# facebookresearch/brainmagick

Measured on AMD Instinct MI355X. Metric: segments/s, 208-ch x 360-sample SimpleConv + ClipLoss training step, higher is better.
Workload: dtype f32 (fp32-accurate: operands split into 2 scaled f16 planes, 3 MFMA products, fp32 accumulate; same parity tolerances as exact fp32, see DESIGN.md §2); 1 GPU; cfg2: gwilliams2022-shaped MEG C=208 T=360, F=120 features, 27 subjects, clip_conv SimpleConv (8985590 params) + ClipLoss + Adam; batch_per_gpu=256, global_batch=256, negatives=local, parallelism=dp1, comm=none, rccl_world=1, candidate_gather=none, distinct_batches=8

## Files before the change

### brainmagick_amd/csrc/core.hip

```cpp
#include "bm_common.h"
#include <stdarg.h>
#include <stdlib.h>

thread_local char bm_err_buf[512] = {0};

int bm_set_error(int code, const char* fmt, ...) {
    va_list ap;
    va_start(ap, fmt);
    vsnprintf(bm_err_buf, sizeof(bm_err_buf), fmt, ap);
    va_end(ap);
    return code;
}

int bm_check_launch(const char* what) {
    hipError_t e = hipGetLastError();
    if (e != hipSuccess) return bm_set_error((int)e, "%s: launch failed: %s", what, hipGetErrorString(e));
    return BM_OK;
}

extern "C" const char* bm_last_error(void) { return bm_err_buf; }
extern "C" int bm_version(void) { return 110; }

extern "C" int bm_device_count(void) {
    int n = 0;
    hipError_t e = hipGetDeviceCount(&n);
    if (e != hipSuccess) { bm_set_error((int)e, "hipGetDeviceCount: %s", hipGetErrorString(e)); return -1; }
    return n;
}

__global__ __launch_bounds__(1024) void amax_finalize_kernel(const float* __restrict__ ws, int n, float* __restrict__ out) {
    __shared__ float sh[16];
    float m = 0.f;
    for (int i = threadIdx.x; i < n; i += 1024) m = fmaxf(m, ws[i]);
    m = bm_wave_max(m);
    if ((threadIdx.x & 63) == 0) sh[threadIdx.x >> 6] = m;
    __syncthreads();
    if (threadIdx.x < BM_AMAX_SHARDS) {
        float v = 0.f;
        if (threadIdx.x == 0)
            for (int w = 0; w < 16; ++w) v = fmaxf(v, sh[w]);
        out[threadIdx.x] = v;
    }
}

// ... 50 lines not shown
```

### brainmagick_amd/csrc/gemm_nt_h2w.hip

```cpp
#include <cstdlib>
#include "gemm_nt_common.h"

typedef _Float16 f16x8 __attribute__((ext_vector_type(8)));
typedef _Float16 f16x4 __attribute__((ext_vector_type(4)));
typedef unsigned int u32x2 __attribute__((ext_vector_type(2)));

#define HG_K 32
#define HG_XQ (64 + 2)

struct GemmNTArgsH {
    const float* a; long a_sstride; long a_rstride;
    const float* x; long x_sstride; long x_rstride;
    const float* a_amax; const float* x_amax;
    const float* a_row_amax;
    float* part;
    int S, M, Cn, T, dil, nsplit;
    int tiles_m, tiles_c;
    const int* order; const int* seg;
};

__device__ __forceinline__ u32x4 hg_ld128(__amdgpu_buffer_rsrc_t rs, int voff, int soff) {
    return __builtin_amdgcn_raw_buffer_load_b128(rs, voff, soff, 0);
}
__device__ __forceinline__ unsigned hg_ld32(__amdgpu_buffer_rsrc_t rs, int voff) {
    return __builtin_amdgcn_raw_buffer_load_b32(rs, voff, 0, 0);
}

__device__ __forceinline__ void hg_split_store4(const float (&f)[4], float s, char* dst, int plane_bytes) {
    f16x4 h, l;
#pragma unroll
    for (int i = 0; i < 4; ++i) {
        const float xs = f[i] * s;
        const _Float16 a = (_Float16)xs;
        h[i] = a;
        l[i] = (_Float16)(xs - (float)a);
    }
    *reinterpret_cast<u32x2*>(dst) = __builtin_bit_cast(u32x2, h);
    *reinterpret_cast<u32x2*>(dst + plane_bytes) = __builtin_bit_cast(u32x2, l);
}

__device__ __forceinline__ void hg_split_hi(float x0, float x1, float s0, float s1, unsigned& hi) {
    asm("v_fma_mixlo_f16 %0, %1, %3, 0\n\t"
// ... 21 lines not shown
                     :: "memory");
}

template <int NP>
__device__ __forceinline__ void hg_touch(u32x4 (&r)[NP]) {
    if constexpr (NP == 16)
        asm volatile("" :: "v"(r[0]), "v"(r[1]), "v"(r[2]), "v"(r[3]), "v"(r[4]), "v"(r[5]), "v"(r[6]), "v"(r[7]),
                     "v"(r[8]), "v"(r[9]), "v"(r[10]), "v"(r[11]), "v"(r[12]), "v"(r[13]), "v"(r[14]), "v"(r[15]));
    else
        asm volatile("" :: "v"(r[0]), "v"(r[1]), "v"(r[2]), "v"(r[3]), "v"(r[4]), "v"(r[5]), "v"(r[6]), "v"(r[7]),
                     "v"(r[8]), "v"(r[9]), "v"(r[10]), "v"(r[11]));
}

#ifdef HG_TRACE
__device__ long long hg_trace_buf[64 * 4 * 8];
#define HG_T(I_) { __builtin_amdgcn_sched_barrier(0); tr[I_] = __builtin_readcyclecounter(); __builtin_amdgcn_sched_barrier(0); }
extern "C" int bm_debug_trace_read(long long* out) {
    return (int)hipMemcpyFromSymbol(out, HIP_SYMBOL(hg_trace_buf), sizeof(long long) * 64 * 4 * 8);
}
#else
#define HG_T(I_)
#endif

template <int KS, int MW, int NS, bool RS = false, bool TS = false, bool FL = false>
__global__ __launch_bounds__(256, 1) void gemm_nt_h2w_kernel(GemmNTArgsH a) {
    static_assert(!FL || RS, "the flat walk relies on the row-scaled A path (pieces inside or outside a row)");
    static_assert((MW == 5 && NS == 3) || (MW == 4 && NS == 2) || (MW == 4 && NS == 4),
                  "tile variants: 320 x 192, 256 x 128, 256 x 256");
    static_assert(!TS || (KS == 1 && !RS), "the transposed partial tile is the score contraction's");
    static_assert(KS == 1 || NS == 3, "3 taps use the 3 slots");
    constexpr int NA = 2 * MW;
    constexpr int NX = 2 * NS;
    constexpr int NP = NA + NX;
    constexpr int BM = 64 * MW;
    constexpr int BC = KS == 3 ? 64 : 64 * NS;
    constexpr int AQ = BM + 2;
    constexpr int ASLOTS = 4 * AQ;
    constexpr int PLANE = ASLOTS + NS * 4 * HG_XQ;
    constexpr int BUF = 2 * PLANE;
    constexpr int TN = MW * NS;
    constexpr int NXS = KS == 3 ? 3 : 1;
#ifdef HG_TRACE
    const long long t_kernel0 = __builtin_readcyclecounter();
    long long t_loop0 = t_kernel0, t_loop1 = t_kernel0;
#endif
    extern __shared__ __attribute__((aligned(16))) float smem[];
    u32x4* lds = reinterpret_cast<u32x4*>(smem);
    const int tid = threadIdx.x;
    const int lane = tid & 63;
    const int wave = __builtin_amdgcn_readfirstlane(tid >> 6);
    const int wm = wave >> 1, wc = wave & 1;
    const int nl = lane & 31, h = lane >> 5;

    int id = bm_xcd_remap(blockIdx.x, gridDim.x);
    const int tm = id % a.tiles_m; id /= a.tiles_m;
    const int tc = id % a.tiles_c; id /= a.tiles_c;
    const int split = id % a.nsplit;
    const int grp = id / a.nsplit;
    const int m0 = tm * BM, c0 = tc * BC;
    const int s_first = a.seg ? a.seg[grp] : 0;
    const int s_count = a.seg ? a.seg[grp + 1] - s_first : a.S;
#define HG_SEG(K_) (a.order ? a.order[s_first + (K_)] : s_first + (K_))

    const int cps = (a.T + HG_K - 1) / HG_K;
    const long nchunks = FL ? ((long)a.S * a.T + HG_K - 1) / HG_K : (long)s_count * cps;
    const long q_begin = nchunks * split / a.nsplit;
    const long q_end = nchunks * (split + 1) / a.nsplit;
    const int nst = (int)(q_end - q_begin);
    const int halo = KS == 3 ? a.dil : 0;
    const int a_bytes = (int)(((FL ? (long)(a.S - 1) * a.a_sstride : 0) + (long)(a.M - 1) * a.a_rstride + a.T) * 4);
    const int x_bytes = (int)(((FL ? (long)(a.S - 1) * a.x_sstride : 0) + (long)(a.Cn - 1) * a.x_rstride + a.T) * 4);
    float sa, sa_inv, sx, sx_inv;
    bm_scale_from_amax(bm_amax_load(a.a_amax), sa, sa_inv);
    bm_scale_from_amax(bm_amax_load(a.x_amax), sx, sx_inv);

    const int row32 = tid >> 3, pl = tid & 7;
    int offa[NA], offx[NX];
#pragma unroll
    for (int i = 0; i < NA; ++i) {
        const int m = m0 + 32 * i + row32;
        offa[i] = m < a.M ? (m * (int)a.a_rstride + 4 * pl) * 4 : 0x7f000000;
    }
#pragma unroll
    for (int q = 0; q < NX; ++q) {
        const int c = c0 + (KS == 3 ? 0 : 64 * (q >> 1)) + 32 * (q & 1) + row32;
        offx[q] = c < a.Cn ? (c * (int)a.x_rstride + 4 * pl) * 4 : 0x7f000000;
    }
    const int ldsa = ((pl >> 1) * AQ + row32) * 16 + (pl & 1) * 8;
    const int ldsx = (ASLOTS + (pl >> 1) * HG_XQ + row32) * 16 + (pl & 1) * 8;

// ... 232 lines not shown
#undef HG_SV
#undef HG_S
#undef HG_SPLIT0
#undef HG_SPLIT_SUB
#undef HG_BOOKKEEPING
#undef HG_SPLIT1
#undef HG_WRITE
#undef HG_READ_A1
#undef HG_READ_B1
#undef HG_READ_A
#undef HG_READ_B

    const long N = (long)a.Cn * KS;
    float* dst = a.part + ((long)grp * a.nsplit + split) * a.M * N;
    if constexpr (RS) {
        __syncthreads();
        for (int i = tid; i < BM; i += 256) {
            float s_unused, inv_m = 0.f;
            if (m0 + i < a.M) bm_scale_from_amax(a.a_row_amax[m0 + i], s_unused, inv_m);
            smem[i] = inv_m;
        }
        __syncthreads();
    }
    if constexpr (TS) {
        const float f = sa_inv * sx_inv;
        float* dstT = a.part + ((long)grp * a.nsplit + split) * a.Cn * a.M;
#pragma unroll
        for (int j = 0; j < NS; ++j) {
            const int c = c0 + 64 * j + wc * 32 + nl;
            if (c < a.Cn) {
#pragma unroll
                for (int mt = 0; mt < MW; ++mt)
#pragma unroll
                    for (int q = 0; q < 4; ++q) {
                        const int m = m0 + wm * (MW * 32) + mt * 32 + 8 * q + 4 * h;
                        if (m < a.M)
                            *reinterpret_cast<float4*>(dstT + (long)c * a.M + m) =
                                float4{acc[mt][j][4 * q] * f, acc[mt][j][4 * q + 1] * f, acc[mt][j][4 * q + 2] * f,
                                       acc[mt][j][4 * q + 3] * f};
                    }
            }
        }
        return;
    }
#pragma unroll
    for (int mt = 0; mt < MW; ++mt) {
// ... 10 lines not shown
                        p[0] = acc[mt][0][r] * f;
                        p[1] = acc[mt][1][r] * f;
                        p[2] = acc[mt][2][r] * f;
                    }
                } else {
#pragma unroll
                    for (int j = 0; j < NS; ++j) {
                        const int c = c0 + 64 * j + wc * 32 + nl;
                        if (c < a.Cn) dst[(long)m * N + c] = acc[mt][j][r] * f;
                    }
                }
            }
        }
    }
#ifdef HG_TRACE
    asm volatile("s_waitcnt vmcnt(0)" ::: "memory");
    if (blockIdx.x < 64 && lane == 0) {
        long long* o = hg_trace_buf + (blockIdx.x * 4 + wave) * 8;
        o[2] = t_loop0 - t_kernel0;
        o[3] = t_loop1 - t_loop0;
        o[6] = (long long)__builtin_readcyclecounter() - t_loop1;
    }
#endif
}

static int hg_family(int S, int G, int M, int Cn, int T, int KS, int dil, bool ordered) {
    if (KS != 3 && KS != 1) return 0;
    if ((G != 1 || ordered) && KS != 1) return 0;
    if (dil < 1 || dil > 32 || T < 2 * HG_K) return 0;
    if ((long)S * ((T + HG_K - 1) / HG_K) < 32L * G) return 0;
    const long work = (long)M * Cn;
    const long pad53 = (long)cdiv(M, 320) * 320 * cdiv(Cn, KS == 3 ? 64 : 192) * (KS == 3 ? 64 : 192);
    if (KS == 3) return pad53 * 4 <= work * 5 ? 1 : 0;
    const long pad42 = (long)cdiv(M, 256) * 256 * cdiv(Cn, 128) * 128;
    if (pad42 < pad53 && pad42 <= work * 2) return 2;
    return pad53 <= work * 2 ? 1 : 0;
}

extern "C" int bm_gemm_nt_h2_covers(int M, int Cn, int KS, int S, int T, int G, int dil, int ordered) {
    return hg_family(S, G, M, Cn, T, KS, dil, ordered != 0) ? 1 : 0;
}

extern "C" int bm_gemm_nt_h2_suggest_splits(int M, int Cn, int KS, int S, int T) {
    return bm_gemm_nt_h2_suggest_splits_grouped(M, Cn, KS, S, T, 1);
}
extern "C" int bm_gemm_nt_h2_suggest_splits_grouped(int M, int Cn, int KS, int S, int T, int G) {
// ... 3 lines not shown
    const long chunks = (long)(S / G > 0 ? S / G : 1) * ((T + HG_K - 1) / HG_K);
    long want = 256 / tiles;
    if (want > chunks / 8) want = chunks / 8;
    if (want < 1) want = 1;
    return (int)want;
}

template <int KS, int MW, int NS, bool RS = false, bool TS = false, bool FL = false>
static int launch_gemm_nt_h2w(GemmNTArgsH g, hipStream_t stream, int ngroups = 1) {
    constexpr int PLANE = 4 * (64 * MW + 2) + NS * 4 * HG_XQ;
    const size_t lds = (size_t)2 * 2 * PLANE * 16;
    static bool attr_set = false;
    if (!attr_set) {
        hipError_t e = hipFuncSetAttribute(reinterpret_cast<const void*>(gemm_nt_h2w_kernel<KS, MW, NS, RS, TS, FL>),
                                           hipFuncAttributeMaxDynamicSharedMemorySize, (int)lds);
        if (e != hipSuccess) return bm_set_error((int)e, "gemm_nt_h2w: hipFuncSetAttribute: %s", hipGetErrorString(e));
        attr_set = true;
    }
    g.tiles_m = cdiv(g.M, 64 * MW);
    g.tiles_c = cdiv(g.Cn, KS == 3 ? 64 : 64 * NS);
    const long nblocks = (long)g.tiles_m * g.tiles_c * g.nsplit * ngroups;
    hipLaunchKernelGGL((gemm_nt_h2w_kernel<KS, MW, NS, RS, TS, FL>), dim3((unsigned)nblocks), dim3(256), lds, stream, g);
    return bm_check_launch("gemm_nt_h2w");
}

static int gemm_nt_h2_impl(const float* a, long a_sstride, long a_rstride, const float* a_amax, const float* a_row_amax,
                           const float* x, long x_sstride, long x_rstride, const float* x_amax, float* part, int S,
                           int M, int Cn, int T, int KS, int dil, int nsplit, void* stream,
                           const int* order = nullptr, const int* seg = nullptr, int G = 1) {
    BM_REQUIRE(a && x && part && a_amax && x_amax, "gemm_nt_h2: null pointer");
    BM_REQUIRE(M > 0 && Cn > 0 && T > 0 && nsplit > 0 && S >= 0, "gemm_nt_h2: bad dims");
    BM_REQUIRE(G >= 1 && (G == 1 || seg), "gemm_nt_h2: a grouped call needs seg[]");
    const bool grouped = seg != nullptr || order != nullptr;
    const int fam = hg_family(S, G, M, Cn, T, KS, dil, grouped);
    BM_REQUIRE(fam != 0, "gemm_nt_h2: shape not covered (M=%d Cn=%d T=%d KS=%d dil=%d)", M, Cn, T, KS, dil);
    if (((long)(M - 1) * a_rstride + T) * 4 >= 0x7f000000L || ((long)(Cn - 1) * x_rstride + T) * 4 >= 0x7f000000L)
        return bm_gemm_nt_x3(a, a_sstride, a_rstride, x, x_sstride, x_rstride, order, seg, part, S, G, M, Cn, T,
                             KS, dil, nsplit, stream);
    GemmNTArgsH g;
    g.a = a; g.a_sstride = a_sstride; g.a_rstride = a_rstride; g.a_amax = a_amax;
    g.x = x; g.x_sstride = x_sstride; g.x_rstride = x_rstride; g.x_amax = x_amax;
    g.a_row_amax = a_row_amax;
    g.part = part; g.S = S; g.M = M; g.Cn = Cn; g.T = T; g.dil = dil; g.nsplit = nsplit;
    g.order = order; g.seg = seg;
    hipStream_t s = (hipStream_t)stream;
    if (grouped) {
        if (fam == 2) return launch_gemm_nt_h2w<1, 4, 2>(g, s, G);
        return launch_gemm_nt_h2w<1, 5, 3>(g, s, G);
    }
    const bool rs = a_row_amax && fam == 1 && T % 4 == 0 && a_rstride % 4 == 0 && a_sstride % 4 == 0;
    const bool flat = rs && KS == 3 && T % HG_K != 0 && T >= 2 * HG_K && S > 1 &&
                      ((long)(S - 1) * a_sstride + (long)(M - 1) * a_rstride + T) * 4 < 0x7f000000L &&
                      ((long)(S - 1) * x_sstride + (long)(Cn - 1) * x_rstride + T) * 4 < 0x7f000000L &&
                      a_sstride >= T && x_sstride >= T && x_sstride % 4 == 0;
    if (flat) return launch_gemm_nt_h2w<3, 5, 3, true, false, true>(g, s);
    if (KS == 3) return rs ? launch_gemm_nt_h2w<3, 5, 3, true>(g, s) : launch_gemm_nt_h2w<3, 5, 3>(g, s);
    if (fam == 2) return launch_gemm_nt_h2w<1, 4, 2>(g, s);
    return rs ? launch_gemm_nt_h2w<1, 5, 3, true>(g, s) : launch_gemm_nt_h2w<1, 5, 3>(g, s);
}

extern "C" int bm_gemm_nt_h2(const float* a, long a_sstride, long a_rstride, const float* a_amax, const float* x,
                             long x_sstride, long x_rstride, const float* x_amax, float* part, int S, int M, int Cn,
                             int T, int KS, int dil, int nsplit, void* stream) {
    return gemm_nt_h2_impl(a, a_sstride, a_rstride, a_amax, nullptr, x, x_sstride, x_rstride, x_amax, part, S, M, Cn, T,
                           KS, dil, nsplit, stream);
}

extern "C" int bm_gemm_nt_h2_rows(const float* a, long a_sstride, long a_rstride, const float* a_amax,
                                  const float* a_row_amax, const float* x, long x_sstride, long x_rstride,
                                  const float* x_amax, float* part, int S, int M, int Cn, int T, int KS, int dil,
                                  int nsplit, void* stream) {
    return gemm_nt_h2_impl(a, a_sstride, a_rstride, a_amax, a_row_amax, x, x_sstride, x_rstride, x_amax, part, S, M, Cn,
                           T, KS, dil, nsplit, stream);
}

extern "C" int bm_gemm_nt_h2_grouped(const float* a, long a_sstride, long a_rstride, const float* a_amax, const float* x,
                                     long x_sstride, long x_rstride, const float* x_amax, const int* order,
                                     const int* seg, float* part, int S, int G, int M, int Cn, int T, int nsplit,
                                     void* stream) {
    return gemm_nt_h2_impl(a, a_sstride, a_rstride, a_amax, nullptr, x, x_sstride, x_rstride, x_amax, part, S, M, Cn, T,
                           1, 1, nsplit, stream, order, seg, G);
}

static int clip_scores_wide(int B, int Bc, long K) {
    const long tiles = (long)cdiv(Bc, 256) * cdiv(B, 256);
    const long chunks = (K + HG_K - 1) / HG_K;
    long splits = 256 / tiles;
    if (splits < 1) splits = 1;
    return chunks / splits >= 16;
}

extern "C" int bm_clip_scores_h2_covers(int B, int Bc, long K) {
    if (B <= 0 || Bc <= 0 || Bc % 4 != 0 || K < 16 * HG_K || K >= 0x7fffffffL) return 0;
    if (((long)(Bc - 1) * K + K) * 4 >= 0x7f000000L || ((long)(B - 1) * K + K) * 4 >= 0x7f000000L) return 0;
    const int bc = clip_scores_wide(B, Bc, K) ? 256 : 128;
    return (long)cdiv(Bc, 256) * 256 * cdiv(B, bc) * bc * 2 <= (long)B * Bc * 3;
}

extern "C" int bm_clip_scores_h2_suggest_splits(int B, int Bc, long K) {
    const int bc = clip_scores_wide(B, Bc, K) ? 256 : 128;
    const int tiles = cdiv(Bc, 256) * cdiv(B, bc);
    const long chunks = (K + HG_K - 1) / HG_K;
    long want = 256 / tiles;
    if (want > chunks / 4) want = chunks / 4;
// ... 17 lines not shown
```

### brainmagick_amd/functional.py

```python

import torch

from . import hip_ops as H



ACT_CODES = {"none": H.ACT_NONE, "gelu": H.ACT_GELU, "relu": H.ACT_RELU, "leaky": H.ACT_LEAKY}


def _c(t: torch.Tensor) -> torch.Tensor:
    return t if t.is_contiguous() else t.contiguous()


_arange_cache = {}


def _arange_i32(n: int, device, repeat: int = 1) -> torch.Tensor:
    key = (n, repeat, device.type, device.index)
    t = _arange_cache.get(key)
    if t is None:
        if len(_arange_cache) > 64:
            _arange_cache.clear()
        t = torch.arange(n, dtype=torch.int32, device=device)
        if repeat != 1:
            t = t.repeat(repeat)
        if device.type == "cuda":
            torch.cuda.current_stream(device).synchronize()
        _arange_cache[key] = t
    return t


def _conv_weight_grads(dy, x, weight, KS, dil, transposed_weight):
    dst = H.grad_destination(weight)
    B, M, T = dy.shape
    Cin = x.shape[1]
    if transposed_weight:
        out = dst if dst is not None else torch.empty(weight.shape, device=dy.device, dtype=torch.float32)
        H.gemm_nt(x, dy, B, Cin, M, T, 1, 1, out=out.view(1, Cin, M, 1))
        return out.view(weight.shape) if dst is not None else out
    if dst is not None:
        H.gemm_nt(dy, x, B, M, Cin, T, KS, dil, out=dst.view(1, M, Cin, KS))
        return dst.view(weight.shape)
    return H.gemm_nt(dy, x, B, M, Cin, T, KS, dil).view(weight.shape)


def _layer_forward(x, weight, geom, res=None, **kw):
    dil, transposed, stride, pad = geom
    if pad is not None:
        assert res is None, "the strided family has no fused residual"
        KS = weight.shape[2]
        M = weight.shape[1] if transposed else weight.shape[0]
        Tout = H.conv_out_len(x.shape[2], KS, stride, dil, pad, transposed)
        wp = H.pack_strided_rows_second(weight) if transposed else H.pack_strided_rows_first(weight)
        return H.conv_strided(x, wp, M, Tout, KS, stride, dil, pad, transposed, **kw)
    assert stride == 1
    if transposed:
        Cin, M, KS = weight.shape
        assert KS == 1, "ConvTranspose1d is only supported with kernel 1 (simpleconv.py:189)"
        wp = H.pack_weights(weight, 1, M, Cin, 1, 0, 1, M, 0, shape=(x.shape[2], dil))
    else:
        M, Cin, KS = weight.shape
        wp = H.pack_conv_fwd(weight, (x.shape[2], dil))
    if kw.get("want_stats") and getattr(wp, "_bm_mode", "") != "f16x2":
        pre, out, _ = H.conv_nn(x, wp, M, KS, dil, res=res, **dict(kw, want_stats=False))
# ... 500 lines not shown
```

### brainmagick_amd/hip_ops.py

```python
import ctypes
import typing as tp

import torch

from ._lib import lib, check, BmHipError

ACT_NONE, ACT_GELU, ACT_RELU, ACT_LEAKY = 0, 1, 2, 3
BKC = 16

import os as _os
DEFAULT_COMPUTE_DTYPE = "f16x2"
COMPUTE_DTYPES = ("f32", "f32x3", "f16x2")
_compute_dtype = _os.environ.get("BM_COMPUTE_DTYPE", DEFAULT_COMPUTE_DTYPE)
if _compute_dtype not in COMPUTE_DTYPES:
    raise ValueError(f"BM_COMPUTE_DTYPE must be one of {COMPUTE_DTYPES}, got {_compute_dtype!r}")


def set_compute_dtype(name: str):
    global _compute_dtype
    if name not in COMPUTE_DTYPES:
        raise ValueError(f"compute dtype must be one of {COMPUTE_DTYPES}, got {name!r}")
    _compute_dtype = name


def get_compute_dtype() -> str:
    return _compute_dtype


class KernelTimer:

    def __init__(self):
        self.records: tp.List[tp.Tuple[str, float, torch.cuda.Event, torch.cuda.Event]] = []

    def launch(self, name: str, flops: float, fn):
        start = torch.cuda.Event(enable_timing=True)
        end = torch.cuda.Event(enable_timing=True)
        start.record()
        out = fn()
        end.record()
        self.records.append((name, flops, start, end))
        return out

    def summary(self) -> tp.Dict[str, tp.Dict[str, float]]:
        samples: tp.Dict[str, tp.List[float]] = {}
        flops_sum: tp.Dict[str, float] = {}
        for name, flops, start, end in self.records:
            samples.setdefault(name, []).append(start.elapsed_time(end))
            flops_sum[name] = flops_sum.get(name, 0.0) + flops
        out = {}
        for name, v in samples.items():
            med = sorted(v)[len(v) // 2]
            kept = [t for t in v if t <= 20.0 * med]
            out[name] = dict(launches=len(v), avg_ms=sum(kept) / len(kept), median_ms=med, max_ms=max(v),
                             outliers=len(v) - len(kept), flops_per_launch=flops_sum[name] / len(v))
        return out


_timer: tp.Optional[KernelTimer] = None
_MODE_SUFFIX = {"f32": "", "f32x3": "_x3", "f16x2": "_h2w"}


def set_kernel_timer(timer: tp.Optional[KernelTimer]):
    global _timer
    _timer = timer


def _timed(label, flops: float, launch):
    if _timer is None:
        return launch()
    return _timer.launch(label() if callable(label) else label, flops, launch)
# ... 509 lines not shown
    if part is not out:
        check(lib().bm_reduce_splits(_p(part), _p(out), G, nsplit, M, Cn, KS, *out_strides,
                                     _stream()), "bm_reduce_splits")
    return out


class _DirectArmed:
    depth = 0

    @property
    def on(self):
        return self.depth > 0


_direct_armed = _DirectArmed()


class direct_grads_armed:

    def __enter__(self):
        _direct_armed.depth += 1
        return self

    def __exit__(self, *exc):
        _direct_armed.depth -= 1
        return False


def grad_destination(param: torch.Tensor) -> tp.Optional[torch.Tensor]:
    dst = getattr(param, "_bm_grad_dst", None)
    if dst is None or dst[1][0] or param.grad is not None or not _direct_armed.on:
        return None
    dst[1][0] = True
    return dst[0]


def gemm_nt_partials(a, x, S, M, Cn, T, a_strides, x_strides, nsplit=None):
    _req(a, "gemm_nt.a")
    _req(x, "gemm_nt.x")
    family, _, nsplit = _nt_plan(M, Cn, 1, S, T, 1, 1, False, a_strides, x_strides, nsplit, partials=True)
    part = torch.empty(nsplit, M, Cn, device=a.device, dtype=torch.float32)
    _nt_launch(family, "clip_scores:gemm_nt{}", a, x, part, S, 1, M, Cn, T, 1, 1, a_strides, x_strides, None, None, nsplit)
    return part


def sum_over_batch(x: torch.Tensor) -> torch.Tensor:
    _req(x, "sum_over_batch.x")
    B = x.shape[0]
    out = torch.empty(x.shape[1:], device=x.device, dtype=torch.float32)
    check(lib().bm_sum_over_batch(_p(x), _p(out), B, out.numel(), _stream()), "bm_sum_over_batch")
    return out


def bn_finalize(stats, count: int, gamma, beta, running_mean, running_var, num_batches,
                momentum: float, eps: float):
    _req(stats, "bn_finalize.stats")
    channel_major = getattr(stats, "_bm_channel_major", False)
# ... 676 lines not shown
```

### include/bm_hip.h

```cpp
#ifndef BM_HIP_H
#define BM_HIP_H
#ifdef __cplusplus
extern "C" {
#endif

#define BM_ACT_NONE 0
#define BM_ACT_GELU 1
#define BM_ACT_RELU 2
#define BM_ACT_LEAKY 3

int bm_version(void);
const char* bm_last_error(void);
int bm_device_count(void);

int bm_conv_mt_for(int M);
int bm_conv_mpad(int M);
int bm_conv_stats_tiles(int B, int T);
long bm_packed_weight_elems(int G, int M, int Cin, int KS);
int bm_pack_weights(const float* src, float* dst, int G, int M, int Cin, int KS, long sg, long sm,
                    long sc, long sj, int flip, const float* alpha_ptr, void* stream);
int bm_group_by_index(const long* idx, int B, int G, int* order, int* seg, int* err_flag, void* stream);
int bm_index_to_i32(const long* idx, int B, int G, int* out, int* err_flag, void* stream);
int bm_reduce_splits(const float* part, float* out, int G, int nsplit, int M, int Cn, int KS, long sg,
                     long sm, long sc, long sj, void* stream);
// ... 52 lines not shown
int bm_amax_ws_elems(void);
int bm_amax(const float* x, long n, float* out, float* amax_ws, void* stream);
int bm_amax_checked(const float* x, long n, float* out, float* amax_ws, int* nonfinite_flag, void* stream);
int bm_conv_h2_stats_tiles(int B, int T);
int bm_conv1d_nn_h2(const float* x, long x_bstride, const float* x_amax, const void* wpacked, const int* widx,
                    const float* bias, long bias_gstride, const float* ep_scale, const float* ep_shift, const float* res,
                    long res_bstride, float* y_pre, float* y_out, long y_bstride, float* stats, int B, int Cin,
                    int M, int T, int KS, int dil, int act, float leak, int G, float* y_amax_out, float* amax_ws,
                    void* stream);

int bm_gemm_nt_h2_covers(int M, int Cn, int KS, int S, int T, int G, int dil, int ordered);
int bm_gemm_nt_h2_suggest_splits(int M, int Cn, int KS, int S, int T);
int bm_gemm_nt_h2(const float* a, long a_sstride, long a_rstride, const float* a_amax, const float* x,
                  long x_sstride, long x_rstride, const float* x_amax, float* part, int S, int M, int Cn, int T,
                  int KS, int dil, int nsplit, void* stream);
int bm_gemm_nt_h2_rows(const float* a, long a_sstride, long a_rstride, const float* a_amax, const float* a_row_amax,
                       const float* x, long x_sstride, long x_rstride, const float* x_amax, float* part, int S,
                       int M, int Cn, int T, int KS, int dil, int nsplit, void* stream);

int bm_gemm_nt_h2_grouped(const float* a, long a_sstride, long a_rstride, const float* a_amax, const float* x,
                          long x_sstride, long x_rstride, const float* x_amax, const int* order, const int* seg,
                          float* part, int S, int G, int M, int Cn, int T, int nsplit, void* stream);
int bm_gemm_nt_h2_suggest_splits_grouped(int M, int Cn, int KS, int S, int T, int G);

int bm_clip_scores_h2_covers(int B, int Bc, long K);
int bm_clip_scores_h2_suggest_splits(int B, int Bc, long K);
int bm_clip_scores_h2(const float* est, const float* est_amax, const float* cand, const float* cand_amax, float* part,
                      int B, int Bc, long K, int nsplit, void* stream);

int bm_gemm_nt_suggest_splits(int M, int Cn, int KS, int S, int T, int G);
int bm_clip_suggest_splits(int M, int Cn, int S, int T);
int bm_gemm_nt(const float* a, long a_sstride, long a_rstride, const float* x, long x_sstride,
               long x_rstride, const int* order, const int* seg, float* part, int S, int G, int M,
               int Cn, int T, int KS, int dil, int nsplit, void* stream);

int bm_bn_finalize(const float* stats, int ntiles, int C, long count, const float* gamma,
                   const float* beta, float* running_mean, float* running_var, long* num_batches,
                   float momentum, float eps, float* mean, float* invstd, float* scale, float* shift,
                   void* stream);
int bm_bn_finalize_cm(const float* stats, int ntiles, int C, long count, const float* gamma,
                   const float* beta, float* running_mean, float* running_var, long* num_batches,
                   float momentum, float eps, float* mean, float* invstd, float* scale, float* shift,
                   void* stream);
int bm_bn_eval_affine(int C, const float* gamma, const float* beta, const float* running_mean,
                      const float* running_var, float eps, float* mean, float* invstd, float* scale,
                      float* shift, void* stream);
// ... 125 lines not shown
```

Before: 17320 segments/s.

## Batch 3-tap conv weight-gradient GEMMs into one persistent multi-job launch

```diff
diff --git a/brainmagick_amd/csrc/core.hip b/brainmagick_amd/csrc/core.hip
--- a/brainmagick_amd/csrc/core.hip
+++ b/brainmagick_amd/csrc/core.hip
@@ -19,7 +19,7 @@
 }
 
 extern "C" const char* bm_last_error(void) { return bm_err_buf; }
-extern "C" int bm_version(void) { return 110; }
+extern "C" int bm_version(void) { return 111; }
 
 extern "C" int bm_device_count(void) {
     int n = 0;
diff --git a/brainmagick_amd/csrc/gemm_nt_h2w.hip b/brainmagick_amd/csrc/gemm_nt_h2w.hip
--- a/brainmagick_amd/csrc/gemm_nt_h2w.hip
+++ b/brainmagick_amd/csrc/gemm_nt_h2w.hip
@@ -1,5 +1,7 @@
 #include <cstdlib>
+#include <cstring>
 #include "gemm_nt_common.h"
+#include "wgrad_batch_plan.h"
 
 typedef _Float16 f16x8 __attribute__((ext_vector_type(8)));
 typedef _Float16 f16x4 __attribute__((ext_vector_type(4)));
@@ -18,6 +20,28 @@
     int tiles_m, tiles_c;
     const int* order; const int* seg;
 };
+
+#define HG_MAX_JOBS 24
+#define HG_TILE_ELEMS (320 * 192)
+struct HgJob {
+    const float* a; const float* x; const float* a_amax; const float* x_amax; const float* a_row_amax;
+    float* out;
+    int M, Cn, dil;
+    int out_sm, out_sc, out_sj;
+};
+struct GemmNTBatchArgsH {
+    HgJob job[HG_MAX_JOBS];
+    const int* pieces;
+    const int* team_range;
+    const int* units;
+    const int* unit_range;
+    float* part;
+    int S, T, tiles_c, nunits;
+};
+template <bool JOBS> struct HgKernelArgs { typedef GemmNTArgsH type; };
+template <> struct HgKernelArgs<true> { typedef GemmNTBatchArgsH type; };
+__device__ __forceinline__ const GemmNTArgsH& hg_args_of(const GemmNTArgsH& ka, const GemmNTArgsH&) { return ka; }
+__device__ __forceinline__ const GemmNTArgsH& hg_args_of(const GemmNTBatchArgsH&, const GemmNTArgsH& ja) { return ja; }
 
 __device__ __forceinline__ u32x4 hg_ld128(__amdgpu_buffer_rsrc_t rs, int voff, int soff) {
     return __builtin_amdgcn_raw_buffer_load_b128(rs, voff, soff, 0);
@@ -85,9 +109,10 @@
 #define HG_T(I_)
 #endif
 
-template <int KS, int MW, int NS, bool RS = false, bool TS = false, bool FL = false>
-__global__ __launch_bounds__(256, 1) void gemm_nt_h2w_kernel(GemmNTArgsH a) {
+template <int KS, int MW, int NS, bool RS = false, bool TS = false, bool FL = false, bool JOBS = false>
+__global__ __launch_bounds__(256, 1) void gemm_nt_h2w_kernel(typename HgKernelArgs<JOBS>::type ka) {
     static_assert(!FL || RS, "the flat walk relies on the row-scaled A path (pieces inside or outside a row)");
+    static_assert(!JOBS || (KS == 3 && MW == 5 && RS && !TS), "batched: the row-scaled 3-tap weight gradients");
     static_assert((MW == 5 && NS == 3) || (MW == 4 && NS == 2) || (MW == 4 && NS == 4),
                   "tile variants: 320 x 192, 256 x 128, 256 x 256");
     static_assert(!TS || (KS == 1 && !RS), "the transposed partial tile is the score contraction's");
@@ -116,10 +141,37 @@
     const int nl = lane & 31, h = lane >> 5;
 
     int id = bm_xcd_remap(blockIdx.x, gridDim.x);
-    const int tm = id % a.tiles_m; id /= a.tiles_m;
-    const int tc = id % a.tiles_c; id /= a.tiles_c;
-    const int split = id % a.nsplit;
-    const int grp = id / a.nsplit;
+    int pc_begin = 0, pc_end = 1, tc_team = 0;
+    if constexpr (JOBS) {
+        tc_team = id % ka.tiles_c;
+        const int team = id / ka.tiles_c;
+        pc_begin = ka.team_range[team];
+        pc_end = ka.team_range[team + 1];
+    }
+    for (int pc = pc_begin; pc < pc_end; ++pc) {
+    GemmNTArgsH ja;
+    int tm, tc, split, grp, pq_begin = 0, pq_end = 0;
+    if constexpr (JOBS) {
+        __syncthreads();
+        const int unit = ka.pieces[4 * pc];
+        pq_begin = ka.pieces[4 * pc + 1];
+        pq_end = ka.pieces[4 * pc + 2];
+        const HgJob& jb = ka.job[ka.units[2 * unit]];
+        ja.a = jb.a; ja.a_sstride = (long)jb.M * ka.T; ja.a_rstride = ka.T;
+        ja.x = jb.x; ja.x_sstride = (long)jb.Cn * ka.T; ja.x_rstride = ka.T;
+        ja.a_amax = jb.a_amax; ja.x_amax = jb.x_amax; ja.a_row_amax = jb.a_row_amax;
+        ja.part = nullptr; ja.S = ka.S; ja.M = jb.M; ja.Cn = jb.Cn; ja.T = ka.T; ja.dil = jb.dil; ja.nsplit = 1;
+        ja.tiles_m = 1; ja.tiles_c = ka.tiles_c; ja.order = nullptr; ja.seg = nullptr;
+        tm = ka.units[2 * unit + 1]; tc = tc_team; split = 0; grp = 0;
+    }
+    const GemmNTArgsH& a = hg_args_of(ka, ja);
+    if constexpr (!JOBS) {
+        int id_ = id;
+        tm = id_ % a.tiles_m; id_ /= a.tiles_m;
+        tc = id_ % a.tiles_c; id_ /= a.tiles_c;
+        split = id_ % a.nsplit;
+        grp = id_ / a.nsplit;
+    }
     const int m0 = tm * BM, c0 = tc * BC;
     const int s_first = a.seg ? a.seg[grp] : 0;
     const int s_count = a.seg ? a.seg[grp + 1] - s_first : a.S;
@@ -127,8 +179,8 @@
 
     const int cps = (a.T + HG_K - 1) / HG_K;
     const long nchunks = FL ? ((long)a.S * a.T + HG_K - 1) / HG_K : (long)s_count * cps;
-    const long q_begin = nchunks * split / a.nsplit;
-    const long q_end = nchunks * (split + 1) / a.nsplit;
+    const long q_begin = JOBS ? (long)pq_begin : nchunks * split / a.nsplit;
+    const long q_end = JOBS ? (long)pq_end : nchunks * (split + 1) / a.nsplit;
     const int nst = (int)(q_end - q_begin);
     const int halo = KS == 3 ? a.dil : 0;
     const int a_bytes = (int)(((FL ? (long)(a.S - 1) * a.a_sstride : 0) + (long)(a.M - 1) * a.a_rstride + a.T) * 4);
@@ -407,6 +459,27 @@
         }
         __syncthreads();
     }
+    if constexpr (JOBS) {
+        float* tile = ka.part + ((long)pc * ka.tiles_c + tc) * HG_TILE_ELEMS;
+        const int cl = wc * 32 + nl;
+        int lane_off = (wm * (MW * 32) + 4 * h) * 192 + cl * 3;
+        asm volatile("" : "+v"(lane_off));
+#pragma unroll
+        for (int mt = 0; mt < MW; ++mt) {
+#pragma unroll
+            for (int r = 0; r < 16; ++r) {
+                const int ml = wm * (MW * 32) + mt * 32 + (r & 3) + 8 * (r >> 2) + 4 * h;
+                if (m0 + ml < a.M && c0 + cl < a.Cn) {
+                    const float f = smem[ml] * sx_inv;
+                    float* p = tile + lane_off + (mt * 32 + (r & 3) + 8 * (r >> 2)) * 192;
+                    p[0] = acc[mt][0][r] * f;
+                    p[1] = acc[mt][1][r] * f;
+                    p[2] = acc[mt][2][r] * f;
+                }
+            }
+        }
+        continue;
+    }
     if constexpr (TS) {
         const float f = sa_inv * sx_inv;
         float* dstT = a.part + ((long)grp * a.nsplit + split) * a.Cn * a.M;
@@ -463,6 +536,8 @@
         o[6] = (long long)__builtin_readcyclecounter() - t_loop1;
     }
 #endif
+    if constexpr (!JOBS) return;
+    }
 }
 
 static int hg_family(int S, int G, int M, int Cn, int T, int KS, int dil, bool ordered) {
@@ -512,6 +587,13 @@
     const long nblocks = (long)g.tiles_m * g.tiles_c * g.nsplit * ngroups;
     hipLaunchKernelGGL((gemm_nt_h2w_kernel<KS, MW, NS, RS, TS, FL>), dim3((unsigned)nblocks), dim3(256), lds, stream, g);
     return bm_check_launch("gemm_nt_h2w");
+}
+
+static bool hg_flat_ok(int S, int M, int Cn, int T, long a_sstride, long a_rstride, long x_sstride, long x_rstride) {
+    return T % HG_K != 0 && T >= 2 * HG_K && S > 1 &&
+           ((long)(S - 1) * a_sstride + (long)(M - 1) * a_rstride + T) * 4 < 0x7f000000L &&
+           ((long)(S - 1) * x_sstride + (long)(Cn - 1) * x_rstride + T) * 4 < 0x7f000000L &&
+           a_sstride >= T && x_sstride >= T && x_sstride % 4 == 0;
 }
 
 static int gemm_nt_h2_impl(const float* a, long a_sstride, long a_rstride, const float* a_amax, const float* a_row_amax,
@@ -539,10 +621,7 @@
         return launch_gemm_nt_h2w<1, 5, 3>(g, s, G);
     }
     const bool rs = a_row_amax && fam == 1 && T % 4 == 0 && a_rstride % 4 == 0 && a_sstride % 4 == 0;
-    const bool flat = rs && KS == 3 && T % HG_K != 0 && T >= 2 * HG_K && S > 1 &&
-                      ((long)(S - 1) * a_sstride + (long)(M - 1) * a_rstride + T) * 4 < 0x7f000000L &&
-                      ((long)(S - 1) * x_sstride + (long)(Cn - 1) * x_rstride + T) * 4 < 0x7f000000L &&
-                      a_sstride >= T && x_sstride >= T && x_sstride % 4 == 0;
+    const bool flat = rs && KS == 3 && hg_flat_ok(S, M, Cn, T, a_sstride, a_rstride, x_sstride, x_rstride);
     if (flat) return launch_gemm_nt_h2w<3, 5, 3, true, false, true>(g, s);
     if (KS == 3) return rs ? launch_gemm_nt_h2w<3, 5, 3, true>(g, s) : launch_gemm_nt_h2w<3, 5, 3>(g, s);
     if (fam == 2) return launch_gemm_nt_h2w<1, 4, 2>(g, s);
@@ -570,6 +649,146 @@
                                      void* stream) {
     return gemm_nt_h2_impl(a, a_sstride, a_rstride, a_amax, nullptr, x, x_sstride, x_rstride, x_amax, part, S, M, Cn, T,
                            1, 1, nsplit, stream, order, seg, G);
+}
+
+__global__ __launch_bounds__(256) void wgrad_batch_fold_kernel(GemmNTBatchArgsH ka) {
+    const int unit = blockIdx.z, tc = blockIdx.y;
+    const HgJob& jb = ka.job[ka.units[2 * unit]];
+    const int m0 = ka.units[2 * unit + 1] * 320, c0 = tc * 64;
+    const int p0 = ka.unit_range[unit], p1 = ka.unit_range[unit + 1];
+    const int rows = jb.M - m0 < 320 ? jb.M - m0 : 320;
+    const int ncol = (jb.Cn - c0 < 64 ? jb.Cn - c0 : 64) * 3;
+    const bool vec = jb.out_sj == 1 && jb.out_sc == 3 && jb.out_sm % 4 == 0 && ((uintptr_t)jb.out % 16) == 0;
+    const long pstride = (long)ka.tiles_c * HG_TILE_ELEMS;
+    for (int i = threadIdx.x; i < 16 * 48; i += 256) {
+        const int ml = blockIdx.x * 16 + i / 48, col = (i % 48) * 4;
+        if (ml >= rows || col >= ncol) continue;
+        const float* p = ka.part + ((long)p0 * ka.tiles_c + tc) * HG_TILE_ELEMS + ml * 192 + col;
+        float4 s = make_float4(0.f, 0.f, 0.f, 0.f);
+        int k = p0;
+        for (; k + 4 <= p1; k += 4, p += 4 * pstride) {
+            float4 v[4];
+#pragma unroll
+            for (int u = 0; u < 4; ++u) v[u] = *reinterpret_cast<const float4*>(p + u * pstride);
+#pragma unroll
+            for (int u = 0; u < 4; ++u) { s.x += v[u].x; s.y += v[u].y; s.z += v[u].z; s.w += v[u].w; }
+        }
+        for (; k < p1; ++k, p += pstride) {
+            const float4 v = *reinterpret_cast<const float4*>(p);
+            s.x += v.x; s.y += v.y; s.z += v.z; s.w += v.w;
+        }
+        float* o = jb.out + (long)(m0 + ml) * jb.out_sm;
+        if (vec && col + 4 <= ncol) {
+            *reinterpret_cast<float4*>(o + c0 * 3 + col) = s;
+        } else {
+            const float sv[4] = {s.x, s.y, s.z, s.w};
+#pragma unroll
+            for (int e = 0; e < 4; ++e) {
+                const int n = col + e;
+                if (n < ncol) o[(long)(c0 + n / 3) * jb.out_sc + (long)(n % 3) * jb.out_sj] = sv[e];
+            }
+        }
+    }
+}
+
+extern "C" int bm_wgrad_batch_walk(int S, int M, int Cn, int T, int dil) {
+    if (S < 1 || M < 1 || Cn < 1 || T < 1) return 0;
+    if (hg_family(S, 1, M, Cn, T, 3, dil, false) != 1 || T % 4 != 0) return 0;
+    if (((long)(M - 1) * T + T) * 4 >= 0x7f000000L || ((long)(Cn - 1) * T + T) * 4 >= 0x7f000000L) return 0;
+    return hg_flat_ok(S, M, Cn, T, (long)M * T, T, (long)Cn * T, T) ? 2 : 1;
+}
+
+extern "C" long bm_wgrad_batch_chunks(int S, int T, int walk) {
+    return walk == 2 ? ((long)S * T + HG_K - 1) / HG_K : (long)S * ((T + HG_K - 1) / HG_K);
+}
+
+extern "C" int bm_wgrad_batch_max_jobs(void) { return HG_MAX_JOBS; }
+
+extern "C" long bm_wgrad_batch_plan(const int* tiles_m, int njobs, int tiles_c, long nchunks, int nwg_max, int cap,
+                                    int* pieces, long max_pieces, int* team_range, int* unit_range, int* units) {
+    return bm_wgrad_plan_impl(tiles_m, njobs, tiles_c, nchunks, nwg_max > 0 ? nwg_max : 256, cap, pieces, max_pieces,
+                              team_range, unit_range, units);
+}
+
+extern "C" long bm_wgrad_batch_workspace_bytes(long npieces, int tiles_c) {
+    return npieces * tiles_c * (long)HG_TILE_ELEMS * 4;
+}
+
+extern "C" int bm_wgrad_batch_job_bytes(void) { return (int)sizeof(HgJob); }
+
+extern "C" int bm_wgrad_batch_job_fill(void* job, const float* a, const float* a_amax, const float* a_row_amax,
+                                       const float* x, const float* x_amax, float* out, int M, int Cn, int dil,
+                                       long out_sm, long out_sc, long out_sj) {
+    if (!job || !a || !a_amax || !a_row_amax || !x || !x_amax || !out || M < 1 || Cn < 1 || dil < 1) return -1;
+    if (out_sm < 0 || out_sc < 0 || out_sj < 0 || out_sm > 0x7fffffffL || out_sc > 0x7fffffffL || out_sj > 0x7fffffffL)
+        return -1;
+    HgJob jb;
+    jb.a = a; jb.x = x; jb.a_amax = a_amax; jb.x_amax = x_amax; jb.a_row_amax = a_row_amax; jb.out = out;
+    jb.M = M; jb.Cn = Cn; jb.dil = dil; jb.out_sm = (int)out_sm; jb.out_sc = (int)out_sc; jb.out_sj = (int)out_sj;
+    memcpy(job, &jb, sizeof(jb));
+    return 0;
+}
+
+template <bool FL>
+static int launch_wgrad_batch(const GemmNTBatchArgsH& g, int nteams, hipStream_t stream) {
+    constexpr int PLANE = 4 * (64 * 5 + 2) + 3 * 4 * HG_XQ;
+    const size_t lds = (size_t)2 * 2 * PLANE * 16;
+    static bool attr_set = false;
+    if (!attr_set) {
+        hipError_t e = hipFuncSetAttribute(reinterpret_cast<const void*>(gemm_nt_h2w_kernel<3, 5, 3, true, false, FL, true>),
+                                           hipFuncAttributeMaxDynamicSharedMemorySize, (int)lds);
+        if (e != hipSuccess) return bm_set_error((int)e, "wgrad_batch: hipFuncSetAttribute: %s", hipGetErrorString(e));
+        attr_set = true;
+    }
+    hipLaunchKernelGGL((gemm_nt_h2w_kernel<3, 5, 3, true, false, FL, true>), dim3((unsigned)(nteams * g.tiles_c)),
+                       dim3(256), lds, stream, g);
+    return bm_check_launch("wgrad_batch");
+}
+
+extern "C" int bm_wgrad_batch(const void* jobs, int njobs, int S, int T, int walk, const int* plan_host,
+                              const int* plan_dev, int npieces, int nteams, int nunits, int tiles_c, float* part,
+                              long part_bytes, void* stream) {
+    BM_REQUIRE(jobs && plan_host && plan_dev && part, "wgrad_batch: null pointer");
+    BM_REQUIRE(njobs >= 1 && njobs <= HG_MAX_JOBS, "wgrad_batch: %d jobs (1 .. %d)", njobs, HG_MAX_JOBS);
+    BM_REQUIRE(walk == 1 || walk == 2, "wgrad_batch: walk %d", walk);
+    BM_REQUIRE(npieces >= 1 && nteams >= 1 && nunits >= njobs && tiles_c >= 1 && (long)nteams * tiles_c <= 65536,
+               "wgrad_batch: bad plan dims");
+    BM_REQUIRE(part_bytes >= bm_wgrad_batch_workspace_bytes(npieces, tiles_c), "wgrad_batch: workspace too small");
+    GemmNTBatchArgsH g;
+    memset(&g, 0, sizeof(g));
+    memcpy(g.job, jobs, sizeof(HgJob) * njobs);
+    for (int j = 0; j < njobs; ++j) {
+        const HgJob& jb = g.job[j];
+        BM_REQUIRE(jb.a && jb.x && jb.a_amax && jb.x_amax && jb.a_row_amax && jb.out, "wgrad_batch: job %d: null pointer", j);
+        BM_REQUIRE(bm_wgrad_batch_walk(S, jb.M, jb.Cn, T, jb.dil) == walk && cdiv(jb.Cn, 64) == tiles_c,
+                   "wgrad_batch: job %d (M=%d Cn=%d dil=%d) does not belong to this batch", j, jb.M, jb.Cn, jb.dil);
+    }
+    const long nchunks = bm_wgrad_batch_chunks(S, T, walk);
+    const int* pieces = plan_host;
+    const int* team_range = pieces + 4L * npieces;
+    const int* units = team_range + nteams + 1;
+    const int* unit_range = units + 2L * nunits;
+    bool ok = team_range[0] == 0 && team_range[nteams] == npieces && unit_range[0] == 0 && unit_range[nunits] == npieces;
+    for (int k = 0; ok && k < nteams; ++k) ok = team_range[k] <= team_range[k + 1];
+    for (int u = 0; ok && u < nunits; ++u) {
+        const int j = units[2 * u];
+        ok = j >= 0 && j < njobs && units[2 * u + 1] >= 0 && units[2 * u + 1] < cdiv(g.job[j].M, 320) &&
+             unit_range[u] <= unit_range[u + 1];
+        for (int p = unit_range[u]; ok && p < unit_range[u + 1]; ++p)
+            ok = p < npieces && pieces[4 * p] == u && pieces[4 * p + 1] >= 0 && pieces[4 * p + 1] < pieces[4 * p + 2] &&
+                 pieces[4 * p + 2] <= nchunks;
+    }
+    BM_REQUIRE(ok, "wgrad_batch: inconsistent plan tables");
+    g.pieces = plan_dev;
+    g.team_range = plan_dev + 4L * npieces;
+    g.units = g.team_range + nteams + 1;
+    g.unit_range = g.units + 2L * nunits;
+    g.part = part; g.S = S; g.T = T; g.tiles_c = tiles_c; g.nunits = nunits;
+    hipStream_t s = (hipStream_t)stream;
+    const int rc = walk == 2 ? launch_wgrad_batch<true>(g, nteams, s) : launch_wgrad_batch<false>(g, nteams, s);
+    if (rc != BM_OK) return rc;
+    hipLaunchKernelGGL(wgrad_batch_fold_kernel, dim3(20, tiles_c, nunits), dim3(256), 0, s, g);
+    return bm_check_launch("wgrad_batch_fold");
 }
 
 static int clip_scores_wide(int B, int Bc, long K) {
diff --git a/brainmagick_amd/csrc/wgrad_batch_plan.h b/brainmagick_amd/csrc/wgrad_batch_plan.h
--- /dev/null
+++ b/brainmagick_amd/csrc/wgrad_batch_plan.h
@@ -0,0 +1,41 @@
+#pragma once
+
+static inline long bm_wgrad_plan_impl(const int* tiles_m, int njobs, int tiles_c, long nchunks, int nwg_max, int cap,
+                                      int* pieces, long max_pieces, int* team_range, int* unit_range, int* units) {
+    if (!tiles_m || njobs < 1 || tiles_c < 1 || nchunks < 1 || nchunks > 0x7fffffffL || nwg_max < tiles_c || cap < 0)
+        return -1;
+    long nunits = 0;
+    for (int j = 0; j < njobs; ++j) {
+        if (tiles_m[j] < 1 || tiles_m[j] > 0x10000) return -1;
+        for (int b = 0; b < tiles_m[j]; ++b, ++nunits)
+            if (units) { units[2 * nunits] = j; units[2 * nunits + 1] = b; }
+    }
+    if (nunits > 0x10000) return -1;
+    const long nteams = nwg_max / tiles_c;
+    const long total = nunits * nchunks;
+    if (nteams > 0xffff) return -1;
+    long np = 0, next_unit = 0;
+    for (long k = 0; k < nteams; ++k) {
+        if (team_range) team_range[k] = (int)np;
+        const long hi = total * (k + 1) / nteams;
+        long pos = total * k / nteams;
+        while (pos < hi) {
+            const long u = pos / nchunks, q = pos - u * nchunks;
+            long end = (u + 1) * nchunks < hi ? (u + 1) * nchunks : hi;
+            if (cap > 0 && pos + cap < end) end = pos + cap;
+            if (np >= 0x7fffffffL) return -1;
+            if (pieces) {
+                if (np >= max_pieces) return -2;
+                pieces[4 * np] = (int)u; pieces[4 * np + 1] = (int)q; pieces[4 * np + 2] = (int)(q + (end - pos));
+                pieces[4 * np + 3] = 0;
+            }
+            for (; unit_range && next_unit <= u; ++next_unit) unit_range[next_unit] = (int)np;
+            if (!unit_range) next_unit = u + 1;
+            ++np;
+            pos = end;
+        }
+    }
+    if (team_range) team_range[nteams] = (int)np;
+    if (unit_range) unit_range[nunits] = (int)np;
+    return np;
+}
diff --git a/brainmagick_amd/functional.py b/brainmagick_amd/functional.py
--- a/brainmagick_amd/functional.py
+++ b/brainmagick_amd/functional.py
@@ -39,7 +39,8 @@
         H.gemm_nt(x, dy, B, Cin, M, T, 1, 1, out=out.view(1, Cin, M, 1))
         return out.view(weight.shape) if dst is not None else out
     if dst is not None:
-        H.gemm_nt(dy, x, B, M, Cin, T, KS, dil, out=dst.view(1, M, Cin, KS))
+        if KS != 3 or not H.wgrad_batch_enqueue(dy, x, dst, B, M, Cin, T, dil):
+            H.gemm_nt(dy, x, B, M, Cin, T, KS, dil, out=dst.view(1, M, Cin, KS))
         return dst.view(weight.shape)
     return H.gemm_nt(dy, x, B, M, Cin, T, KS, dil).view(weight.shape)
 
diff --git a/brainmagick_amd/hip_ops.py b/brainmagick_amd/hip_ops.py
--- a/brainmagick_amd/hip_ops.py
+++ b/brainmagick_amd/hip_ops.py
@@ -41,11 +41,21 @@
         self.records.append((name, flops, start, end))
         return out
 
+    def launch_shared(self, name: str, flops: tp.Sequence[float], fn):
+        start = torch.cuda.Event(enable_timing=True)
+        end = torch.cuda.Event(enable_timing=True)
+        start.record()
+        out = fn()
+        end.record()
+        total = float(sum(flops)) or 1.0
+        self.records.extend((name, f, start, end, f / total) for f in flops)
+        return out
+
     def summary(self) -> tp.Dict[str, tp.Dict[str, float]]:
         samples: tp.Dict[str, tp.List[float]] = {}
         flops_sum: tp.Dict[str, float] = {}
-        for name, flops, start, end in self.records:
-            samples.setdefault(name, []).append(start.elapsed_time(end))
+        for name, flops, start, end, *share in self.records:
+            samples.setdefault(name, []).append(start.elapsed_time(end) * (share[0] if share else 1.0))
             flops_sum[name] = flops_sum.get(name, 0.0) + flops
         out = {}
         for name, v in samples.items():
@@ -601,17 +611,141 @@
         _direct_armed.depth += 1
         return self
 
-    def __exit__(self, *exc):
+    def __exit__(self, exc_type, exc, tb):
         _direct_armed.depth -= 1
+        if _direct_armed.depth == 0:
+            if exc_type is None:
+                wgrad_batch_flush()
+            else:
+                _wgrad_queue.clear()
         return False
 
 
 def grad_destination(param: torch.Tensor) -> tp.Optional[torch.Tensor]:
     dst = getattr(param, "_bm_grad_dst", None)
+    if dst is not None and dst[1][0] and _wgrad_queue:
+        wgrad_batch_flush()
     if dst is None or dst[1][0] or param.grad is not None or not _direct_armed.on:
         return None
     dst[1][0] = True
     return dst[0]
+
+
+_WGRAD_BATCH = _os.environ.get("BM_WGRAD_BATCH", "1") != "0"
+WGRAD_BATCH_CAP = 512
+_wgrad_queue: tp.List[dict] = []
+_wgrad_plans: tp.Dict[tuple, dict] = {}
+wgrad_batch_launches = 0
+
+
+def set_wgrad_batch(on: bool) -> bool:
+    global _WGRAD_BATCH
+    prev, _WGRAD_BATCH = _WGRAD_BATCH, bool(on)
+    return prev
+
+
+def wgrad_batch_job(dy: torch.Tensor, x: torch.Tensor, dst: torch.Tensor, S: int, M: int, Cn: int, T: int,
+                    dil: int) -> tp.Optional[dict]:
+    if _compute_dtype != "f16x2":
+        return None
+    if not (dy.is_cuda and dy.dtype == torch.float32 and dy.is_contiguous() and x.dtype == torch.float32 and
+            x.is_contiguous() and dst.is_contiguous() and dst.numel() == M * Cn * 3):
+        return None
+    family, swapped, _ = _nt_plan(M, Cn, 3, S, T, 1, dil, False, (M * T, T), (Cn * T, T))
+    if family != "h2_rows" or swapped:
+        return None
+    walk = lib().bm_wgrad_batch_walk(S, M, Cn, T, dil)
+    a_rows = row_amax_of(dy)
+    if walk == 0 or a_rows is None or a_rows.numel() != M:
+        return None
+    _touched(dst)
+    bucket = dst._base if dst._base is not None else dst
+    return dict(dy=dy, x=x, a_amax=amax(dy), x_amax=amax(x), a_rows=a_rows, bucket=bucket,
+                offset=dst.storage_offset(), S=S, M=M, Cn=Cn, T=T, dil=dil, walk=walk)
+
+
+def wgrad_batch_enqueue(dy: torch.Tensor, x: torch.Tensor, dst: torch.Tensor, S: int, M: int, Cn: int, T: int,
+                        dil: int) -> bool:
+    if not (_WGRAD_BATCH and _direct_armed.on):
+        return False
+    job = wgrad_batch_job(dy, x, dst, S, M, Cn, T, dil)
+    if job is None:
+        return False
+    _wgrad_queue.append(job)
+    return True
+
+
+def _wgrad_plan(tiles_m: tp.Tuple[int, ...], tiles_c: int, nchunks: int, nwg_max: int, cap: int, device) -> dict:
+    key = (tiles_m, tiles_c, nchunks, nwg_max, cap, device.type, device.index)
+    plan = _wgrad_plans.get(key)
+    if plan is None:
+        L = lib()
+        if len(_wgrad_plans) > 64:
+            _wgrad_plans.clear()
+        n = len(tiles_m)
+        tm = (ctypes.c_int * n)(*tiles_m)
+        npieces = L.bm_wgrad_batch_plan(tm, n, tiles_c, nchunks, nwg_max, cap, None, 0, None, None, None)
+        if npieces < 1:
+            raise BmHipError(f"bm_wgrad_batch_plan: bad arguments {key!r}")
+        nteams, nunits = (nwg_max if nwg_max > 0 else 256) // tiles_c, sum(tiles_m)
+        table = (ctypes.c_int * (4 * npieces + nteams + 1 + 2 * nunits + nunits + 1))()
+        at = lambda i: ctypes.c_void_p(ctypes.addressof(table) + 4 * i)
+        got = L.bm_wgrad_batch_plan(tm, n, tiles_c, nchunks, nwg_max, cap, at(0), npieces, at(4 * npieces),
+                                    at(4 * npieces + nteams + 1 + 2 * nunits), at(4 * npieces + nteams + 1))
+        assert got == npieces, (got, npieces)
+        dev = torch.frombuffer(bytearray(table), dtype=torch.int32).to(device)
+        plan = _wgrad_plans[key] = dict(host=table, dev=dev, npieces=npieces, nteams=nteams, nunits=nunits)
+    return plan
+
+
+def wgrad_batch_run(jobs: tp.List[dict], nwg_max: int = 0, cap: tp.Optional[int] = None):
+    global wgrad_batch_launches
+    L = lib()
+    j0 = jobs[0]
+    S, T, walk, device = j0["S"], j0["T"], j0["walk"], j0["dy"].device
+    tiles_c = -(-j0["Cn"] // 64)
+    cap = WGRAD_BATCH_CAP if cap is None else cap
+    plan = _wgrad_plan(tuple(-(-j["M"] // 320) for j in jobs), tiles_c, L.bm_wgrad_batch_chunks(S, T, walk), nwg_max,
+                       cap, device)
+    nb = L.bm_wgrad_batch_job_bytes()
+    host = ctypes.create_string_buffer(nb * len(jobs))
+    for i, j in enumerate(jobs):
+        out = j["bucket"].view(-1)[j["offset"]:j["offset"] + j["M"] * j["Cn"] * 3]
+        if L.bm_wgrad_batch_job_fill(ctypes.c_void_p(ctypes.addressof(host) + i * nb), _p(j["dy"]), _p(j["a_amax"]),
+                                     _p(j["a_rows"]), _p(j["x"]), _p(j["x_amax"]), _p(out), j["M"], j["Cn"], j["dil"],
+                                     j["Cn"] * 3, 3, 1) != 0:
+            raise BmHipError("bm_wgrad_batch_job_fill: bad arguments")
+    nbytes = L.bm_wgrad_batch_workspace_bytes(plan["npieces"], tiles_c)
+    part = torch.empty(nbytes // 4, device=device, dtype=torch.float32)
+
+    def launch():
+        check(L.bm_wgrad_batch(host, len(jobs), S, T, walk, plan["host"], _p(plan["dev"]), plan["npieces"],
+                               plan["nteams"], plan["nunits"], tiles_c, _p(part), nbytes, _stream()), "bm_wgrad_batch")
+    if _timer is None:
+        launch()
+    else:
+        _timer.launch_shared("gemm_nt_h2w_kernel<KS=3> batched", [2.0 * S * T * j["M"] * j["Cn"] * 3 for j in jobs], launch)
+    wgrad_batch_launches += 1
+
+
+def wgrad_batch_flush():
+    jobs = list(_wgrad_queue)
+    _wgrad_queue.clear()
+    if not jobs:
+        return
+    groups: tp.Dict[tuple, tp.List[dict]] = {}
+    for j in jobs:
+        groups.setdefault((-(-j["Cn"] // 64), j["S"], j["T"], j["walk"], j["dy"].device), []).append(j)
+    max_jobs = lib().bm_wgrad_batch_max_jobs()
+    for group in groups.values():
+        for lo in range(0, len(group), max_jobs):
+            chunk = group[lo:lo + max_jobs]
+            if len(chunk) > 1:
+                wgrad_batch_run(chunk)
+                continue
+            j = chunk[0]
+            out = j["bucket"].view(-1)[j["offset"]:j["offset"] + j["M"] * j["Cn"] * 3]
+            gemm_nt(j["dy"], j["x"], j["S"], j["M"], j["Cn"], j["T"], 3, j["dil"], out=out.view(1, j["M"], j["Cn"], 3))
 
 
 def gemm_nt_partials(a, x, S, M, Cn, T, a_strides, x_strides, nsplit=None):
diff --git a/include/bm_hip.h b/include/bm_hip.h
--- a/include/bm_hip.h
+++ b/include/bm_hip.h
@@ -98,6 +98,19 @@
                           long x_sstride, long x_rstride, const float* x_amax, const int* order, const int* seg,
                           float* part, int S, int G, int M, int Cn, int T, int nsplit, void* stream);
 int bm_gemm_nt_h2_suggest_splits_grouped(int M, int Cn, int KS, int S, int T, int G);
+
+int bm_wgrad_batch_walk(int S, int M, int Cn, int T, int dil);
+long bm_wgrad_batch_chunks(int S, int T, int walk);
+int bm_wgrad_batch_max_jobs(void);
+long bm_wgrad_batch_plan(const int* tiles_m, int njobs, int tiles_c, long nchunks, int nwg_max, int cap, int* pieces,
+                         long max_pieces, int* team_range, int* unit_range, int* units);
+long bm_wgrad_batch_workspace_bytes(long npieces, int tiles_c);
+int bm_wgrad_batch_job_bytes(void);
+int bm_wgrad_batch_job_fill(void* job, const float* a, const float* a_amax, const float* a_row_amax, const float* x,
+                            const float* x_amax, float* out, int M, int Cn, int dil, long out_sm, long out_sc,
+                            long out_sj);
+int bm_wgrad_batch(const void* jobs, int njobs, int S, int T, int walk, const int* plan_host, const int* plan_dev,
+                   int npieces, int nteams, int nunits, int tiles_c, float* part, long part_bytes, void* stream);
 
 int bm_clip_scores_h2_covers(int B, int Bc, long K);
 int bm_clip_scores_h2_suggest_splits(int B, int Bc, long K);
```

Result: no change. 17490 segments/s (median of 2 runs) (+1.0%).
